# MarchesiGabriele/gpu_matrix_inversion

Measured on AMD Instinct MI355X. Metric: matrices/sec, N=4096 fp32 inversion (Gauss-Jordan, partial pivoting), higher is better.
Workload: dtype f32; 1 GPU; C1 (BASELINE configs[1]): single 4096x4096 fp32 inversion per GPU per step; n=4096, batch_per_gpu=1, algo=blocked, distribution=D_gate (row-permuted U(-1,1)+sqrt(N) I), parallelism=independent matrices sharded over ranks, no data-path collective

## Files before the change

gpu_matrix_inversion_amd/csrc/mi32_rank_bw.h:

```cpp
#pragma once
#include "mi32_blocked_internal.h"
#include <type_traits>
#include <utility>

namespace mi32 {

typedef float rb_float16v __attribute__((ext_vector_type(16)));
typedef float rb_f4v __attribute__((ext_vector_type(4)));

__device__ __forceinline__ void rb_glds16(const float *gsrc, float *lds_wave_base)
{
    __builtin_amdgcn_global_load_lds((const __attribute__((address_space(1))) void *)gsrc,
                                     (__attribute__((address_space(3))) void *)lds_wave_base, 16, 0, 0);
}

template <int BK, int BN = 128>
constexpr size_t rank_bw2_lds_bytes(int kdim)
{
    return (size_t)(2 * BK * (128 + BN)) * sizeof(float) + (size_t)(128 + kdim) * sizeof(int);
}

__device__ __forceinline__ int rb_strip_width(int kdim, int bn)
{
    const int sw = (2 * 1024 * 1024) / (bn * kdim * (int)sizeof(float));
    return sw < 1 ? 1 : sw;
}
__device__ __forceinline__ void rb_tile_of(int id, int TR, int TC, int sw, int &rt, int &ct)
{
    if ((TR & 1) == 0 && (TC & 3) == 0) {
        const int xcd = id & 7, idx = id >> 3;
        const int tr = TR / 2, tc = TC / 4;
        int r, c;
        const int nfull = tc / sw;
        if (idx < nfull * tr * sw) {
            const int strip = idx / (tr * sw), rem = idx - strip * (tr * sw);
            r = rem / sw;
            c = strip * sw + rem % sw;
        } else {
            const int w = tc - nfull * sw, rem = idx - nfull * tr * sw;
            r = rem / w;
            c = nfull * sw + rem % w;
        }
        rt = (xcd >> 2) * tr + r;
        ct = (xcd & 3) * tc + c;
    } else {
        rt = id / TC;
        ct = id % TC;
    }
}

template <int BK, int BN = 128>
__device__ __forceinline__ void rank_bw2_tile(
    const float *__restrict__ src_all, float *__restrict__ dst_all, const float *__restrict__ g_all, size_t gstride,
    const float *__restrict__ gk_all, size_t gkstride, const float *__restrict__ ub_all, const float *__restrict__ xs_all,
    int np, int ld, size_t mstride, int c0, int kdim, const int *__restrict__ map_all, int copy_panel,
    const PanelExport &ex, size_t tstride, int skip_lo, int skip_hi, int b, int rt, int ct, float *rb_smem)
{
    constexpr int BM = 128;
    constexpr int TN = BN / 64;
    constexpr int ND = BK / 8;
    constexpr int NDB = BK * BN / 1024;
    constexpr int KPB = 256 / BN;
    static_assert(NDB >= 1, "B tile smaller than one LDS-DMA per wave");
    float *s_a = rb_smem;
    float *s_b = rb_smem + 2 * BK * 128;
    int *s_map = reinterpret_cast<int *>(rb_smem + 2 * BK * (128 + BN));

    const int tid = threadIdx.x;
    const int lane = tid & 63;
    const int wave = __builtin_amdgcn_readfirstlane(tid >> 6);
    const int wr = wave >> 1, wc = wave & 1;
    const int row0 = rt * BM, col0 = ct * BN;
    const float *src = src_all + (size_t)b * mstride;
    float *dst = dst_all + (size_t)b * mstride;
    const float *gk = gk_all + (size_t)b * gkstride;
    const float *ub = ub_all + (size_t)b * gkstride;
    const float *xs = xs_all + (size_t)b * gkstride;
    const int *map = map_all + (size_t)b * np;

    if (col0 >= skip_lo && col0 < skip_hi) return;
    if (col0 >= c0 && col0 + BN <= c0 + kdim) {
        if (copy_panel) {
            const float *g = g_all + (size_t)b * gstride;
            for (int idx = tid; idx < BM * (BN / 4); idx += 256) {
                const int rr = idx / (BN / 4), c4 = (idx % (BN / 4)) * 4;
                *reinterpret_cast<rb_f4v *>(dst + (size_t)(row0 + rr) * ld + col0 + c4) =
                    *reinterpret_cast<const rb_f4v *>(g + (size_t)(row0 + rr) * ld + col0 + c4);
            }
        }
        return;
    }
    const bool tile_in_block = (row0 >= c0 && row0 < c0 + kdim);

    if (tid < BM) s_map[tid] = map[row0 + tid];
    __syncthreads();

    const int lk = lane >> 5, lc4 = (lane & 31) * 4;
    const int lkb = lane / (BN / 4), lcb4 = (lane % (BN / 4)) * 4;
    const float *a_src = gk + (size_t)lk * np + row0 + lc4;
    const float *b_src = ub + (size_t)lkb * np + col0 + lcb4;

#define MI32_RB_ISSUE(STAGE, KT)                                                                       \
    _Pragma("unroll") for (int i = 0; i < ND; ++i) {                                                   \
        const int kr = 2 * (wave * ND + i);                                                            \
        rb_glds16(a_src + (size_t)((KT) + kr) * np, s_a + ((STAGE) * BK + kr) * 128);                  \
    }                                                                                                  \
    _Pragma("unroll") for (int i = 0; i < NDB; ++i) {                                                  \
        const int kr = KPB * (wave * NDB + i);                                                         \
        rb_glds16(b_src + (size_t)((KT) + kr) * np, s_b + ((STAGE) * BK + kr) * BN);                   \
    }

    const int lcol = lane & 31;
    const int lhalf = lane >> 5;
    const int nk = kdim / BK;
    rb_float16v acc[2][TN];
    if (tile_in_block) {
#pragma unroll
        for (int tm = 0; tm < 2; ++tm)
#pragma unroll
            for (int tn = 0; tn < TN; ++tn) {
                const int col = col0 + wc * (BN / 2) + tn * 32 + lcol;
#pragma unroll
                for (int reg = 0; reg < 16; ++reg) {
                    const int lr = wr * 64 + tm * 32 + (reg & 3) + 8 * (reg >> 2) + 4 * lhalf;
                    acc[tm][tn][reg] = xs[(size_t)(row0 + lr - c0) * np + col];
                }
            }
    } else {
        const unsigned ld4 = (unsigned)ld * 4u;
        const char *srcb = reinterpret_cast<const char *>(src);
#pragma unroll
        for (int tm = 0; tm < 2; ++tm) {
            int4 m4[4];
#pragma unroll
            for (int q = 0; q < 4; ++q) m4[q] = *reinterpret_cast<const int4 *>(&s_map[wr * 64 + tm * 32 + 8 * q + 4 * lhalf]);
#pragma unroll
            for (int tn = 0; tn < TN; ++tn) {
                const unsigned col4 = (unsigned)(col0 + wc * (BN / 2) + tn * 32 + lcol) * 4u;
#pragma unroll
                for (int q = 0; q < 4; ++q) {
                    const int mm[4] = {m4[q].x, m4[q].y, m4[q].z, m4[q].w};
#pragma unroll
                    for (int j = 0; j < 4; ++j)
                        acc[tm][tn][4 * q + j] = __builtin_nontemporal_load(
                            reinterpret_cast<const float *>(srcb + ((unsigned)mm[j] * ld4 + col4)));
                }
            }
        }
    }
    MI32_RB_ISSUE(0, 0)
    for (int t = 0; t < nk; ++t) {
        const int buf = t & 1;
        asm volatile("s_waitcnt vmcnt(0)" ::: "memory");
        __builtin_amdgcn_s_barrier();
        if (t + 1 < nk) { MI32_RB_ISSUE(buf ^ 1, (t + 1) * BK) }
        const float *pa = s_a + buf * BK * 128 + lhalf * 128 + wr * 64 + lcol;
        const float *pb = s_b + buf * BK * BN + lhalf * BN + wc * (BN / 2) + lcol;
        float af[2], bf[TN];
        af[0] = pa[0]; af[1] = pa[32];
#pragma unroll
        for (int tn = 0; tn < TN; ++tn) bf[tn] = pb[tn * 32];
#pragma unroll
        for (int kk = 0; kk < BK; kk += 2) {
            float afn[2] = {0.f, 0.f}, bfn[TN] = {};
            if (kk + 2 < BK) {
                afn[0] = pa[(kk + 2) * 128]; afn[1] = pa[(kk + 2) * 128 + 32];
#pragma unroll
                for (int tn = 0; tn < TN; ++tn) bfn[tn] = pb[(kk + 2) * BN + tn * 32];
            }
            __builtin_amdgcn_sched_barrier(0);
#pragma unroll
            for (int tm = 0; tm < 2; ++tm)
#pragma unroll
                for (int tn = 0; tn < TN; ++tn)
                    acc[tm][tn] = __builtin_amdgcn_mfma_f32_32x32x2f32(af[tm], bf[tn], acc[tm][tn], 0, 0, 0);
#pragma unroll
            for (int q = 0; q < 2; ++q) af[q] = afn[q];
#pragma unroll
            for (int tn = 0; tn < TN; ++tn) bf[tn] = bfn[tn];
        }
    }
#undef MI32_RB_ISSUE

#pragma unroll
    for (int tm = 0; tm < 2; ++tm)
#pragma unroll
        for (int tn = 0; tn < TN; ++tn) {
            const int col = col0 + wc * (BN / 2) + tn * 32 + lcol;
#pragma unroll
            for (int reg = 0; reg < 16; ++reg) {
                const int grow = row0 + wr * 64 + tm * 32 + (reg & 3) + 8 * (reg >> 2) + 4 * lhalf;
                const unsigned boff = (unsigned)grow * ((unsigned)ld * 4u) + (unsigned)col * 4u;
                __builtin_nontemporal_store(acc[tm][tn][reg],
                                            reinterpret_cast<float *>(reinterpret_cast<char *>(dst) + boff));
            }
#pragma unroll
            for (int q = 0; q < 4; ++q)
                panel_export_store4(ex, tstride, b, np, col, row0 + wr * 64 + tm * 32 + 8 * q + 4 * lhalf,
                                    acc[tm][tn][4 * q], acc[tm][tn][4 * q + 1], acc[tm][tn][4 * q + 2],
                                    acc[tm][tn][4 * q + 3]);
        }
}

template <int BK, int WPS, int BN = 128>
__global__ __launch_bounds__(256, WPS) void gj_rank_bw2_kernel(
    const float *__restrict__ src_all, float *__restrict__ dst_all, const float *__restrict__ g_all, size_t gstride,
    const float *__restrict__ gk_all, size_t gkstride, const float *__restrict__ ub_all, const float *__restrict__ xs_all,
    int np, int ld, size_t mstride, int c0, int kdim, const int *__restrict__ map_all, int copy_panel, PanelExport ex,
    size_t tstride, int skip_lo, int skip_hi, const int *__restrict__ guard)
{
    extern __shared__ __attribute__((aligned(16))) float rb_smem[];
    if (guard != nullptr && __builtin_amdgcn_readfirstlane(guard[blockIdx.y]) == MI32_RUNTIME_ERROR) return;
    int rt, ct;
    rb_tile_of(blockIdx.x, np / 128, np / BN, rb_strip_width(kdim, BN), rt, ct);
    rank_bw2_tile<BK, BN>(src_all, dst_all, g_all, gstride, gk_all, gkstride, ub_all, xs_all, np, ld, mstride, c0, kdim,
                          map_all, copy_panel, ex, tstride, skip_lo, skip_hi, blockIdx.y, rt, ct, rb_smem);
}

template <int BK>
__global__ __launch_bounds__(256, 1) void gj_rank_bw2_persistent_kernel(
    const float *__restrict__ src_all, float *__restrict__ dst_all, const float *__restrict__ g_all, size_t gstride,
    const float *__restrict__ gk_all, size_t gkstride, const float *__restrict__ ub_all, const float *__restrict__ xs_all,
    int np, int ld, size_t mstride, int c0, int kdim, const int *__restrict__ map_all, int copy_panel, PanelExport ex,
    size_t tstride, int skip_lo, int skip_hi, const int *__restrict__ guard)
{
    extern __shared__ __attribute__((aligned(16))) float rb_smem[];
    if (guard != nullptr && __builtin_amdgcn_readfirstlane(guard[blockIdx.y]) == MI32_RUNTIME_ERROR) return;
    const int T = np / 128;
    for (int id = blockIdx.x; id < T * T; id += gridDim.x) {
        int rt, ct;
        rb_tile_of(id, T, T, rb_strip_width(kdim, 128), rt, ct);
        rank_bw2_tile<BK, 128>(src_all, dst_all, g_all, gstride, gk_all, gkstride, ub_all, xs_all, np, ld, mstride, c0,
                               kdim, map_all, copy_panel, ex, tstride, skip_lo, skip_hi, blockIdx.y, rt, ct, rb_smem);
        __syncthreads();
    }
}

}
```

Measured before the change: 113.4 matrices/s.

## Use 16-byte C-tile loads and stores via permlane16 swap in rank update

Reorganizes how each lane owns the C tile in the trailing rank update so the accumulator loads and stores become 16-byte vector accesses instead of scalar 4-byte ones. The two column tiles of a wave are interleaved and permlane16_swap is applied before the K loop and after it to move values between MFMA layout and the contiguous memory layout. B fragments are read from LDS as 2-wide vectors to match the remapped columns. The aim is to cut memory instructions on the bandwidth-bound read/modify/write of the trailing matrix, at the cost of extra cross-lane permutes. The persistent kernel keeps the old scalar path.

```diff
diff --git a/gpu_matrix_inversion_amd/csrc/mi32_rank_bw.h b/gpu_matrix_inversion_amd/csrc/mi32_rank_bw.h
--- a/gpu_matrix_inversion_amd/csrc/mi32_rank_bw.h
+++ b/gpu_matrix_inversion_amd/csrc/mi32_rank_bw.h
@@ -7,11 +7,32 @@
 
 typedef float rb_float16v __attribute__((ext_vector_type(16)));
 typedef float rb_f4v __attribute__((ext_vector_type(4)));
+typedef float rb_f2v __attribute__((ext_vector_type(2)));
 
 __device__ __forceinline__ void rb_glds16(const float *gsrc, float *lds_wave_base)
 {
     __builtin_amdgcn_global_load_lds((const __attribute__((address_space(1))) void *)gsrc,
                                      (__attribute__((address_space(3))) void *)lds_wave_base, 16, 0, 0);
+}
+
+__device__ __forceinline__ void rb_swap16(float &lo_rows, float &hi_rows)
+{
+#if defined(__HIP_DEVICE_COMPILE__)
+    const auto r = __builtin_amdgcn_permlane16_swap(__float_as_uint(lo_rows), __float_as_uint(hi_rows), false, false);
+    lo_rows = __uint_as_float(r[0]);
+    hi_rows = __uint_as_float(r[1]);
+#endif
+}
+__device__ __forceinline__ void rb_ctile_turn(rb_float16v (&acc)[2])
+{
+#pragma unroll
+    for (int tn = 0; tn < 2; ++tn)
+#pragma unroll
+        for (int r = 0; r < 16; r += 2) {
+            float a = acc[tn][r], b = acc[tn][r + 1];
+            rb_swap16(a, b);
+            acc[tn][r] = a; acc[tn][r + 1] = b;
+        }
 }
 
 template <int BK, int BN = 128>
@@ -49,7 +70,7 @@
     }
 }
 
-template <int BK, int BN = 128>
+template <int BK, int BN = 128, bool WIDE = true>
 __device__ __forceinline__ void rank_bw2_tile(
     const float *__restrict__ src_all, float *__restrict__ dst_all, const float *__restrict__ g_all, size_t gstride,
     const float *__restrict__ gk_all, size_t gkstride, const float *__restrict__ ub_all, const float *__restrict__ xs_all,
@@ -110,11 +131,42 @@
         rb_glds16(b_src + (size_t)((KT) + kr) * np, s_b + ((STAGE) * BK + kr) * BN);                   \
     }
 
+    static_assert(TN == 2, "the C tile's 16-byte pieces pair the two column tiles of a wave");
     const int lcol = lane & 31;
     const int lhalf = lane >> 5;
     const int nk = kdim / BK;
+    const int lup = lcol >> 4;
+    const int lcm = wc * (BN / 2) + 4 * (lcol & 15);
     rb_float16v acc[2][TN];
-    if (tile_in_block) {
+    if constexpr (WIDE) {
+        const int lr0 = wr * 64 + 4 * lhalf + lup;
+        const char *cbase;
+        unsigned roff[2][8];
+        if (tile_in_block) {
+            cbase = reinterpret_cast<const char *>(xs);
+#pragma unroll
+            for (int tm = 0; tm < 2; ++tm)
+#pragma unroll
+                for (int r = 0; r < 16; r += 2)
+                    roff[tm][r >> 1] = (unsigned)(row0 - c0 + lr0 + tm * 32 + 8 * (r >> 2) + (r & 3)) * ((unsigned)np * 4u);
+        } else {
+            cbase = reinterpret_cast<const char *>(src);
+#pragma unroll
+            for (int tm = 0; tm < 2; ++tm)
+#pragma unroll
+                for (int r = 0; r < 16; r += 2)
+                    roff[tm][r >> 1] = (unsigned)s_map[lr0 + tm * 32 + 8 * (r >> 2) + (r & 3)] * ((unsigned)ld * 4u);
+        }
+        const unsigned coff = (unsigned)(col0 + lcm) * 4u;
+#pragma unroll
+        for (int tm = 0; tm < 2; ++tm)
+#pragma unroll
+            for (int r = 0; r < 16; r += 2) {
+                const rb_f4v v =
+                    __builtin_nontemporal_load(reinterpret_cast<const rb_f4v *>(cbase + (roff[tm][r >> 1] + coff)));
+                acc[tm][0][r] = v[0]; acc[tm][1][r] = v[1]; acc[tm][0][r + 1] = v[2]; acc[tm][1][r + 1] = v[3];
+            }
+    } else if (tile_in_block) {
 #pragma unroll
         for (int tm = 0; tm < 2; ++tm)
 #pragma unroll
@@ -148,25 +200,38 @@
             }
         }
     }
+    if constexpr (WIDE) __builtin_amdgcn_sched_barrier(0);
     MI32_RB_ISSUE(0, 0)
+    if constexpr (WIDE) {
+        __builtin_amdgcn_sched_barrier(0);
+#pragma unroll
+        for (int tm = 0; tm < 2; ++tm) rb_ctile_turn(acc[tm]);
+    }
     for (int t = 0; t < nk; ++t) {
         const int buf = t & 1;
         asm volatile("s_waitcnt vmcnt(0)" ::: "memory");
         __builtin_amdgcn_s_barrier();
         if (t + 1 < nk) { MI32_RB_ISSUE(buf ^ 1, (t + 1) * BK) }
         const float *pa = s_a + buf * BK * 128 + lhalf * 128 + wr * 64 + lcol;
-        const float *pb = s_b + buf * BK * BN + lhalf * BN + wc * (BN / 2) + lcol;
+        const float *pb = s_b + buf * BK * BN + lhalf * BN + (WIDE ? lcm + 2 * lup : wc * (BN / 2) + lcol);
+        auto read_b = [&](int k, float (&v)[TN]) {
+            if constexpr (WIDE) {
+                const rb_f2v v2 = *reinterpret_cast<const rb_f2v *>(pb + k * BN);
+                v[0] = v2[0]; v[1] = v2[1];
+            } else {
+#pragma unroll
+                for (int tn = 0; tn < TN; ++tn) v[tn] = pb[k * BN + tn * 32];
+            }
+        };
         float af[2], bf[TN];
         af[0] = pa[0]; af[1] = pa[32];
-#pragma unroll
-        for (int tn = 0; tn < TN; ++tn) bf[tn] = pb[tn * 32];
+        read_b(0, bf);
 #pragma unroll
         for (int kk = 0; kk < BK; kk += 2) {
             float afn[2] = {0.f, 0.f}, bfn[TN] = {};
             if (kk + 2 < BK) {
                 afn[0] = pa[(kk + 2) * 128]; afn[1] = pa[(kk + 2) * 128 + 32];
-#pragma unroll
-                for (int tn = 0; tn < TN; ++tn) bfn[tn] = pb[(kk + 2) * BN + tn * 32];
+                read_b(kk + 2, bfn);
             }
             __builtin_amdgcn_sched_barrier(0);
 #pragma unroll
@@ -182,24 +247,47 @@
     }
 #undef MI32_RB_ISSUE
 
-#pragma unroll
-    for (int tm = 0; tm < 2; ++tm)
-#pragma unroll
-        for (int tn = 0; tn < TN; ++tn) {
-            const int col = col0 + wc * (BN / 2) + tn * 32 + lcol;
-#pragma unroll
-            for (int reg = 0; reg < 16; ++reg) {
-                const int grow = row0 + wr * 64 + tm * 32 + (reg & 3) + 8 * (reg >> 2) + 4 * lhalf;
-                const unsigned boff = (unsigned)grow * ((unsigned)ld * 4u) + (unsigned)col * 4u;
-                __builtin_nontemporal_store(acc[tm][tn][reg],
-                                            reinterpret_cast<float *>(reinterpret_cast<char *>(dst) + boff));
-            }
-#pragma unroll
-            for (int q = 0; q < 4; ++q)
-                panel_export_store4(ex, tstride, b, np, col, row0 + wr * 64 + tm * 32 + 8 * q + 4 * lhalf,
-                                    acc[tm][tn][4 * q], acc[tm][tn][4 * q + 1], acc[tm][tn][4 * q + 2],
-                                    acc[tm][tn][4 * q + 3]);
-        }
+    if constexpr (WIDE) {
+        const unsigned ld4 = (unsigned)ld * 4u;
+#pragma unroll
+        for (int tm = 0; tm < 2; ++tm) {
+#pragma unroll
+            for (int tn = 0; tn < TN; ++tn)
+#pragma unroll
+                for (int q = 0; q < 4; ++q)
+                    panel_export_store4(ex, tstride, b, np, col0 + lcm + 2 * lup + tn,
+                                        row0 + wr * 64 + tm * 32 + 8 * q + 4 * lhalf, acc[tm][tn][4 * q],
+                                        acc[tm][tn][4 * q + 1], acc[tm][tn][4 * q + 2], acc[tm][tn][4 * q + 3]);
+            rb_ctile_turn(acc[tm]);
+#pragma unroll
+            for (int r = 0; r < 16; r += 2) {
+                const int grow = row0 + wr * 64 + tm * 32 + 8 * (r >> 2) + 4 * lhalf + (r & 3) + lup;
+                rb_f4v v;
+                v[0] = acc[tm][0][r]; v[1] = acc[tm][1][r]; v[2] = acc[tm][0][r + 1]; v[3] = acc[tm][1][r + 1];
+                __builtin_nontemporal_store(v, reinterpret_cast<rb_f4v *>(reinterpret_cast<char *>(dst) +
+                                                                          ((unsigned)grow * ld4 + (unsigned)(col0 + lcm) * 4u)));
+            }
+        }
+    } else {
+#pragma unroll
+        for (int tm = 0; tm < 2; ++tm)
+#pragma unroll
+            for (int tn = 0; tn < TN; ++tn) {
+                const int col = col0 + wc * (BN / 2) + tn * 32 + lcol;
+#pragma unroll
+                for (int reg = 0; reg < 16; ++reg) {
+                    const int grow = row0 + wr * 64 + tm * 32 + (reg & 3) + 8 * (reg >> 2) + 4 * lhalf;
+                    const unsigned boff = (unsigned)grow * ((unsigned)ld * 4u) + (unsigned)col * 4u;
+                    __builtin_nontemporal_store(acc[tm][tn][reg],
+                                                reinterpret_cast<float *>(reinterpret_cast<char *>(dst) + boff));
+                }
+#pragma unroll
+                for (int q = 0; q < 4; ++q)
+                    panel_export_store4(ex, tstride, b, np, col, row0 + wr * 64 + tm * 32 + 8 * q + 4 * lhalf,
+                                        acc[tm][tn][4 * q], acc[tm][tn][4 * q + 1], acc[tm][tn][4 * q + 2],
+                                        acc[tm][tn][4 * q + 3]);
+            }
+    }
 }
 
 template <int BK, int WPS, int BN = 128>
@@ -230,8 +318,8 @@
     for (int id = blockIdx.x; id < T * T; id += gridDim.x) {
         int rt, ct;
         rb_tile_of(id, T, T, rb_strip_width(kdim, 128), rt, ct);
-        rank_bw2_tile<BK, 128>(src_all, dst_all, g_all, gstride, gk_all, gkstride, ub_all, xs_all, np, ld, mstride, c0,
-                               kdim, map_all, copy_panel, ex, tstride, skip_lo, skip_hi, blockIdx.y, rt, ct, rb_smem);
+        rank_bw2_tile<BK, 128, false>(src_all, dst_all, g_all, gstride, gk_all, gkstride, ub_all, xs_all, np, ld, mstride,
+                                      c0, kdim, map_all, copy_panel, ex, tstride, skip_lo, skip_hi, blockIdx.y, rt, ct, rb_smem);
         __syncthreads();
     }
 }
```

New measurement: 113.7 matrices/s, median of 6. No clear change (+0.2%).
